# superlinear-ai/raglite

Measured on AMD Instinct MI355X. Metric: queries/sec, MaxSim 32x1M d=1024 exact top-100, higher is better.
Workload: dtype f32 in / f32 scores: candidate chunks found with the fp16 hi halves of corpus and queries (1 x v_mfma_f32_16x16x32_f16 per multiply, f32 accumulate, rigorous error bound), their scores by v_mfma_f32_16x16x4_f32 (exact f32 products); full-precision fallback: 3 x v_mfma_f32_16x16x32_f16 on hi+lo pairs

## Files before the change

include/raglite_hip.h:

```cpp
#ifndef RAGLITE_HIP_H
#define RAGLITE_HIP_H

#include <stddef.h>
#include <stdint.h>

#ifdef __cplusplus
extern "C" {
#endif

typedef enum {
    RL_OK = 0,
    RL_ERR_INVALID = -1,
    RL_ERR_HIP = -2,
    RL_ERR_UNSUPPORTED = -3,
    RL_ERR_NOMEM = -4
} rl_status;

typedef enum { RL_MEM_HOST = 0, RL_MEM_DEVICE = 1 } rl_mem;
typedef enum {
    RL_ARITH_AUTO = 0,
    RL_ARITH_FP32_EXACT = 1,
    RL_ARITH_F16_SPLIT = 2,
    RL_ARITH_F16_STORED = 3
} rl_arith;
// ... 36 lines not shown

#define RL_IMAGE_PRESPLIT 1u
#define RL_IMAGE_HI 2u
#define RL_IMAGE_HI_PLANE 4u
int rl_index_prepare(rl_index* index, uint32_t images, uint32_t* built, void* stream);

int rl_index_append(rl_index* index, const float* rows, int64_t n_new_rows, const int64_t* new_chunk_sizes,
                    int64_t n_new_chunks, int mem, void* stream);
int rl_index_delete_chunks(rl_index* index, const int64_t* chunk_ordinals, int64_t n, void* stream);
int rl_index_live(rl_index* index, int64_t* live_rows, int64_t* live_chunks, void* stream);
int rl_index_compact(rl_index* index, int64_t* out_remap, int64_t* new_n_rows, int64_t* new_n_chunks, void* stream);

int rl_index_set_arithmetic(rl_index* index, int mode);
int rl_index_arithmetic(rl_index* index, int* in_effect);

typedef enum {
    RL_OPT_HI_SEARCH = 1, RL_OPT_HI_MAXSIM = 2, RL_OPT_HI_PRODUCTS = 3, RL_OPT_PP_PASS = 4, RL_OPT_FUSED_TOPK = 5, RL_OPT_FUSED_HI = 6,
    RL_OPT_FUSED_PP = 7, RL_OPT_FUSED_TOPK_CAP = 8, RL_OPT_FUSED_TOPK_STRIDE = 9, RL_OPT_GEMM_PASS = 10, RL_OPT_QUERY_PAIRS = 11,
    RL_OPT_PLANES_GEMM = 12, RL_OPT_KEEP_IMAGE = 13, RL_OPT_KEEP_HI = 14, RL_OPT_IMAGE_HEADROOM_MB = 15, RL_OPT_ARITHMETIC = 16,
    RL_OPT_EXACT_KTH_THRESHOLD = 17, RL_OPT_FUSED_TWO_ROUNDS = 18, RL_OPT_KEEP_HI_PLANE = 19, RL_OPT_PAIRS_PACKED = 20,
    RL_OPT_F16_EXACT = 21, RL_OPT_LAZY_IMAGES = 22, RL_OPT_FUSED_PP_SAMPLE = 23,
    RL_OPT_LIST_SELECT = 24, RL_OPT_HI_FEW = 25, RL_OPT_TOPK_BLOCK = 26, RL_OPT_HI_PIVOT = 27, RL_OPT_COUNT_ = 28
} rl_option;
enum { RL_OPT_PP_SCHEDULE = 64 };
int rl_set_default_option(int key, int64_t value);
int rl_get_default_option(int key, int64_t* value);
int rl_index_set_option(rl_index* index, int key, int64_t value);
int rl_index_get_option(rl_index* index, int key, int64_t* value);

int rl_search_rows(rl_index* index, const float* queries, int32_t n_queries, int32_t k,
                   float* out_scores, int32_t* out_rows, int mem, void* stream);

int rl_rank_cut_begin(rl_index* index, const float* queries, int32_t n_queries, int mem, void* stream);
int rl_rank_cut_level(rl_index* index, int level, int64_t rank_limit, uint32_t* out_hist, int mem, void* stream);
int rl_rank_cut_level_done(rl_index* index, int level, const uint32_t* hist_sum, int mem, void* stream);
int rl_rank_cut_ties(rl_index* index, int64_t rank_limit, uint32_t* out_ties, int mem, void* stream);
int rl_rank_cut_finish(rl_index* index, int64_t rank_limit, const uint32_t* ties_before, const uint32_t* chunk_filter, int32_t k,
                       float* out_scores, int32_t* out_rows, int mem, void* stream);

int rl_search_chunks(rl_index* index, const float* queries, int32_t n_queries, int32_t num_hits,
                     int32_t k, float* out_scores, int32_t* out_chunks, int32_t* out_counts,
                     int mem, void* stream);

int rl_maxsim_topk(rl_index* index, const float* query_vecs, int32_t nq, int32_t k,
                   float* out_scores, int32_t* out_chunks, int mem, void* stream);
int rl_maxsim_scores(rl_index* index, const float* query_vecs, int32_t nq, float* out_scores,
                     int mem, void* stream);
// ... 106 lines not shown
```

raglite_amd/_abi.py:

```python

from __future__ import annotations

import ctypes as C
import functools
import os
from pathlib import Path

LIB_PATH = Path(os.environ.get("RAGLITE_HIP_LIB") or Path(__file__).resolve().parent / "_lib" / "libraglite_hip.so")

RL_OK, RL_ERR_INVALID, RL_ERR_HIP, RL_ERR_UNSUPPORTED, RL_ERR_NOMEM = 0, -1, -2, -3, -4
MEM_HOST, MEM_DEVICE = 0, 1
METRICS = {"cosine": 0, "dot": 1, "l2": 2}
SYNTH_KINDS = {"uniform": 0, "small_int": 1}
OPTIONS = {
    "hi_search": 1, "hi_maxsim": 2, "hi_products": 3, "pp_pass": 4, "fused_topk": 5, "fused_hi": 6, "fused_pp": 7, "fused_topk_cap": 8,
    "fused_topk_stride": 9, "gemm_pass": 10, "query_pairs": 11, "planes_gemm": 12, "keep_image": 13, "keep_hi": 14,
    "image_headroom_mb": 15, "arithmetic": 16, "exact_kth_threshold": 17, "fused_two_rounds": 18,
    "keep_hi_plane": 19, "pairs_packed": 20, "f16_exact": 21, "lazy_images": 22, "fused_pp_sample": 23, "list_select": 24, "hi_few": 25, "topk_block": 26, "hi_pivot": 27,
}
SCHEDULE_OPTIONS = {"pp_schedule": 64}


def option_key(name: str) -> int:
    return OPTIONS[name] if name in OPTIONS else SCHEDULE_OPTIONS[name]

c_void_p, c_int, c_i32, c_i64, c_u64, c_size_t = C.c_void_p, C.c_int, C.c_int32, C.c_int64, C.c_uint64, C.c_size_t
c_double, c_char_p = C.c_double, C.c_char_p

_SIGNATURES = {
    "rl_version": [],
    "rl_last_error": [],
    "rl_init": [c_int],
    "rl_device_count": [C.POINTER(c_int)],
    "rl_device_info": [c_int, c_char_p, c_int, C.POINTER(c_int), C.POINTER(c_i64)],
    "rl_dev_alloc": [C.POINTER(c_void_p), c_size_t],
    "rl_dev_free": [c_void_p],
    "rl_memcpy_h2d": [c_void_p, c_void_p, c_size_t, c_void_p],
    "rl_memcpy_d2h": [c_void_p, c_void_p, c_size_t, c_void_p],
    "rl_memcpy_d2d": [c_void_p, c_void_p, c_size_t, c_void_p],
    "rl_stream_sync": [c_void_p],
    "rl_synth_fill": [c_void_p, c_i64, c_i64, c_u64, c_int, c_void_p],
    "rl_pool_norm": [c_void_p, c_i64, c_i32, c_void_p, c_void_p, c_i64, c_i32, c_double, c_void_p, c_void_p,
                     c_int, c_void_p],
# ... 142 lines not shown
```

raglite_amd/csrc/api.hip:

```cpp
#include <cmath>
#include <cstdlib>
#include <cstring>
#include <limits>
#include <memory>
#include <mutex>
#include <utility>
#include <vector>

#include "common.h"

namespace rl {

static thread_local std::string g_last_error;
void set_error(const std::string& msg) { g_last_error = msg; }
int fail(int code, const std::string& msg) {
    g_last_error = msg;
    return code;
}

namespace {

hipStream_t as_stream(void* s) { return reinterpret_cast<hipStream_t>(s); }

struct BlockCache {
// ... 157 lines not shown
}
int sync_and_drain(hipStream_t s) {
    RL_HIP(hipStreamSynchronize(s));
    g_pinned.drain();
    return RL_OK;
}
int finish(int mem, hipStream_t s) {
    if (mem == RL_MEM_HOST) return sync_and_drain(s);
    return RL_OK;
}

int scan_mode(int metric) {
    switch (metric) {
        case RL_COSINE: return SCAN_COSINE;
        case RL_DOT: return SCAN_DOT;
        case RL_L2: return SCAN_L2;
        default: return -1;
    }
}

constexpr size_t SCORE_BATCH_BYTES = size_t(8) << 30;

struct Options {
    int64_t v[RL_OPT_PP_SCHEDULE + 1];
    Options() {
        for (auto& x : v) x = 0;
        v[RL_OPT_HI_SEARCH] = v[RL_OPT_HI_MAXSIM] = v[RL_OPT_HI_PRODUCTS] = v[RL_OPT_PP_PASS] = v[RL_OPT_FUSED_TOPK] = v[RL_OPT_FUSED_HI] = 1;
        v[RL_OPT_FUSED_PP] = v[RL_OPT_GEMM_PASS] = v[RL_OPT_QUERY_PAIRS] = v[RL_OPT_PLANES_GEMM] = v[RL_OPT_KEEP_IMAGE] = v[RL_OPT_KEEP_HI] = 1;
        v[RL_OPT_EXACT_KTH_THRESHOLD] = v[RL_OPT_FUSED_TWO_ROUNDS] = v[RL_OPT_KEEP_HI_PLANE] = v[RL_OPT_F16_EXACT] = v[RL_OPT_LAZY_IMAGES] = v[RL_OPT_FUSED_PP_SAMPLE] = v[RL_OPT_LIST_SELECT] = v[RL_OPT_HI_FEW] = 1;
        v[RL_OPT_TOPK_BLOCK] = v[RL_OPT_PAIRS_PACKED] = 2;
        v[RL_OPT_HI_PIVOT] = 1;
        v[RL_OPT_PP_SCHEDULE] = 1;
        v[RL_OPT_IMAGE_HEADROOM_MB] = -1;
        v[RL_OPT_ARITHMETIC] = RL_ARITH_AUTO;
    }
    bool on(int key) const { return v[key] != 0; }
};
std::mutex g_default_opts_mu;
Options g_default_opts;
bool option_key_ok(int key) { return (key >= 1 && key < RL_OPT_COUNT_) || key == RL_OPT_PP_SCHEDULE; }
bool option_value_ok(int key, int64_t value) {
    switch (key) {
        case RL_OPT_HI_SEARCH: case RL_OPT_HI_MAXSIM: case RL_OPT_PP_PASS: case RL_OPT_FUSED_TOPK: case RL_OPT_FUSED_HI: case RL_OPT_FUSED_PP:
        case RL_OPT_GEMM_PASS: case RL_OPT_QUERY_PAIRS: case RL_OPT_PLANES_GEMM: case RL_OPT_KEEP_IMAGE: case RL_OPT_KEEP_HI:
        case RL_OPT_EXACT_KTH_THRESHOLD: case RL_OPT_FUSED_TWO_ROUNDS: case RL_OPT_KEEP_HI_PLANE: case RL_OPT_F16_EXACT: case RL_OPT_LAZY_IMAGES: case RL_OPT_FUSED_PP_SAMPLE: case RL_OPT_LIST_SELECT: case RL_OPT_HI_FEW: case RL_OPT_HI_PIVOT:
        case RL_OPT_PP_SCHEDULE:
            return value == 0 || value == 1;
        case RL_OPT_TOPK_BLOCK: case RL_OPT_PAIRS_PACKED: return value >= 0 && value <= 2;
        case RL_OPT_HI_PRODUCTS: return value == 1 || value == 2;
        case RL_OPT_FUSED_TOPK_CAP: return value >= 0 && value <= MERGE_CAP;
        case RL_OPT_FUSED_TOPK_STRIDE: return value == 0 || (value >= 2 && value <= (int64_t(1) << 20));
        case RL_OPT_IMAGE_HEADROOM_MB: return value >= -1 && value <= (int64_t(1) << 30);
        case RL_OPT_ARITHMETIC: return value == RL_ARITH_AUTO || value == RL_ARITH_FP32_EXACT;
        default: return false;
    }
}

struct Image {
    Pool buf;
    float scale = 0.f;
    int64_t rows = 0;
    void drop() {
        buf.release();
        scale = 0.f;
        rows = 0;
    }
    bool covers(float at, int64_t n_rows) const { return scale > 0.f && scale == at && rows == n_rows && n_rows > 0; }
};
struct NormStats {
    float max_row_norm = 0.f, max_lo_norm = 0.f, max_lo_ratio = 0.f;
// ... 1740 lines not shown
    hb.m = hb.es + (size_t)n * hb.cap;
    hb.es_top = hb.m + n;
    hb.bmax = reinterpret_cast<uint64_t*>((reinterpret_cast<uintptr_t>(hb.es_top + (size_t)n * k) + 7) & ~uintptr_t(7));
}
size_t hi_batch_words(int32_t n, int32_t k) {
    return (size_t)n * k * 3 + (size_t)n * 3 + 16 + (size_t)n * 2048 * 2 + 2 + 2 * pivot_scratch_words(std::min<int32_t>(n, 2));
}
int hi_batch_approx(rl_index* idx, const float* d_q, int32_t nq, int32_t n_queries, int32_t n_gemm, int32_t k, float* sc, int64_t ld, HiBatch& hb,
                    hipStream_t s, bool flag_zeroed = false) {
    hb.one_product = idx->opt.v[RL_OPT_HI_PRODUCTS] == 1;
    hb.exact_kth = idx->opt.on(RL_OPT_EXACT_KTH_THRESHOLD);
    RL_TRY(idx->hibuf.reserve(hi_batch_words(n_gemm, k) * 4));
    hi_batch_layout(idx, n_gemm, k, hb);
    const int32_t cap = hb.cap;
    hb.m_abs = idx->norm_stats.max_lo_norm + sum_eps(idx->dim) * idx->norm_stats.max_row_norm;
    hb.q_unscale = reinterpret_cast<const float*>(idx->qplanes.as<char>() + (size_t)n_queries * idx->dim * 128);
    hb.qsum = hb.q_unscale + 2 * (size_t)n_queries;
    if (!flag_zeroed) RL_HIP(hipMemsetAsync(hb.flag, 0, 16 * sizeof(uint32_t), s));
    (void)cap;
    const bool pp = hb.one_product && idx->dim >= 256 && idx->opt.on(RL_OPT_PP_PASS);
    if (pp)
        RL_TRY(launch_maxsim_pp(approx_image(idx), idx->n_rows, idx->dim, idx->qplanes.p, n_queries, 0, n_gemm, nq, idx->row_to_chunk,
                                idx->offsets, idx->ends.as<uint32_t>(), sc, ld, idx->n_cu, s, approx_scale(idx), nullptr,
                                (int)idx->opt.v[RL_OPT_PP_SCHEDULE]));
    for (int32_t b = 0; !pp && b < n_gemm; b += GEMM_PASS_QUERIES) {
        const int32_t n_q = std::min<int32_t>(GEMM_PASS_QUERIES, n_gemm - b);
        RL_TRY(launch_maxsim_gemm(approx_image(idx), idx->n_rows, idx->dim, idx->qplanes.p, n_queries, b, n_q, nq, idx->row_to_chunk,
                                  idx->offsets, idx->ends.as<uint32_t>(), sc + (int64_t)b * ld, ld, idx->n_cu, s, approx_scale(idx), true,
                                  nullptr, hb.one_product));
    }
    RL_TRY(mask_chunk_scores(idx, sc, n_gemm, ld, hb.filter, s));
    int st_pv = RL_ERR_UNSUPPORTED;
    if (n_gemm < 16 && idx->n_chunks > (int64_t)262144 && idx->opt.on(RL_OPT_HI_PIVOT))
        st_pv = launch_topk_pivot(sc, n_gemm, idx->n_chunks, ld, k, idx->ws, hb.ts, hb.ti, s);
    if (st_pv != RL_OK && st_pv != RL_ERR_UNSUPPORTED) return st_pv;
    if (st_pv == RL_ERR_UNSUPPORTED) RL_TRY(launch_topk(sc, n_gemm, idx->n_chunks, ld, k, idx->ws, hb.ts, hb.ti, s));
    return RL_OK;
}
int hi_batch_fallback(rl_index* idx, const float* d_q, int32_t nq, int32_t n_queries, int32_t n_gemm, int32_t k, float* sc, int64_t ld,
                      const HiBatch& hb, float* d_s, int32_t* d_c, hipStream_t s, bool rows_only = false);
int hi_batch_rescore(rl_index* idx, const float* d_q, int32_t nq, int32_t n_queries, int32_t n_gemm, int32_t k, float* sc, int64_t ld,
                     const HiBatch& hb, float* d_s, int32_t* d_c, hipStream_t s, bool rows_only = false) {
    const size_t q_elems = (size_t)nq * idx->dim;
    const float* rows = idx->E16 ? reinterpret_cast<const float*>(idx->E16) : idx->E;
    const bool rows16 = idx->E16 != nullptr;
    idx->filt = {RL_FILTER_MAXSIM_BATCH, n_gemm, hb.cap, hb.cnt, hb.flag};
    const int packed = (int)idx->opt.v[RL_OPT_PAIRS_PACKED];
// ... 321 lines not shown
    hipStream_t s = as_stream(stream);
    std::lock_guard<std::mutex> lock(idx->mu);
    RL_TRY(use_scratch(idx, s));
    if (idx->has_empty_chunk || idx->n_chunks == 0)
        return fail(RL_ERR_UNSUPPORTED, "rl_maxsim_approx_scores: the approximate pass needs an index without empty chunks");
    RL_TRY(demand_images(idx, approx_image_bit(idx), s));
    if (!approx_image_valid(idx) || nq > 32 || (kernel == 0 && idx->dim < 256))
        return fail(RL_ERR_UNSUPPORTED, "rl_maxsim_approx_scores: this index keeps no HI image (or nq > 32 / dim < 256)");
    DevBuf t_q, t_o, t_b;
    const float* d_q; float* d_o; float* d_b = nullptr;
    const size_t q_elems = (size_t)nq * idx->dim;
    const int64_t ld = idx->n_chunks;
    RL_TRY(stage_in(query_vecs, (size_t)n_queries * q_elems, mem, s, t_q, &d_q));
    RL_TRY(stage_out_begin(out_scores, (size_t)n_queries * ld, mem, t_o, &d_o));
    if (out_bound) RL_TRY(stage_out_begin(out_bound, (size_t)n_queries, mem, t_b, &d_b));
    RL_TRY(idx->qplanes.reserve(query_planes_bytes(idx->dim, n_queries)));
    RL_TRY(launch_query_planes(d_q, idx->dim, nq, (int64_t)q_elems, n_queries, idx->qplanes.p, s));
    const int32_t per = kernel == 0 ? n_queries : GEMM_PASS_QUERIES;
    for (int32_t b = 0; b < n_queries; b += per) {
        const int32_t n_q = std::min<int32_t>(per, n_queries - b);
        if (kernel == 0)
            RL_TRY(launch_maxsim_pp(approx_image(idx), idx->n_rows, idx->dim, idx->qplanes.p, n_queries, b, n_q, nq, idx->row_to_chunk, idx->offsets,
                                    idx->ends.as<uint32_t>(), d_o + (int64_t)b * ld, ld, idx->n_cu, s, approx_scale(idx), nullptr,
                                    (int)idx->opt.v[RL_OPT_PP_SCHEDULE]));
        else
            RL_TRY(launch_maxsim_gemm(approx_image(idx), idx->n_rows, idx->dim, idx->qplanes.p, n_queries, b, n_q, nq, idx->row_to_chunk, idx->offsets,
                                      idx->ends.as<uint32_t>(), d_o + (int64_t)b * ld, ld, idx->n_cu, s, approx_scale(idx), true, nullptr, true));
    }
    if (d_b) {
        const float m_abs = idx->norm_stats.max_lo_norm + sum_eps(idx->dim) * idx->norm_stats.max_row_norm;
        const float* q_unscale = reinterpret_cast<const float*>(idx->qplanes.as<char>() + (size_t)n_queries * idx->dim * 128);
        RL_TRY(idx->hibuf.reserve((size_t)n_queries * 4 * sizeof(float) + 64));
        float* top = idx->hibuf.as<float>();
        float* thr = top + n_queries;
        uint32_t* cnt = reinterpret_cast<uint32_t*>(thr + n_queries);
        uint32_t* flag = cnt + n_queries;
        RL_HIP(hipMemsetAsync(top, 0, (size_t)n_queries * sizeof(float), s));
        RL_HIP(hipMemsetAsync(flag, 0, 16 * sizeof(uint32_t), s));
        RL_TRY(launch_maxsim_threshold(top, n_queries, 1, d_q, nq, idx->dim, (int64_t)q_elems, 1.0f, m_abs, thr, cnt, flag, s, q_unscale,
                                       idx->norm_stats.max_row_norm + idx->norm_stats.max_lo_norm));
        RL_TRY(launch_scale_f32(thr, d_b, -0.5f, n_queries, s));
        idx->filt = {};
    }
    RL_TRY(stage_out_end(out_scores, (size_t)n_queries * ld, mem, s, t_o));
    if (out_bound) RL_TRY(stage_out_end(out_bound, (size_t)n_queries, mem, s, t_b));
    return finish(mem, s);
}
// ... 182 lines not shown
    int st = RL_OK;
    if (kind == 2) {
        st = pairs_prepare(idx, q_dev, nq / 2, (int64_t)(nq / 2) * idx->dim, 2, s);
        if (st != RL_OK) { (void)hipEventDestroy(e0); (void)hipEventDestroy(e1); return st == RL_ERR_UNSUPPORTED ? fail(st, "rl_time_kernel: the pair kernel does not apply to this index / shape") : st; }
    }
    if (kind == 3 || kind == 5 || kind == 6) {
        st = gemm_prepare(idx, q_dev, nq / GEMM_PASS_QUERIES, (int64_t)(nq / GEMM_PASS_QUERIES) * idx->dim, GEMM_PASS_QUERIES, s, true);
        if (st == RL_OK && !image_valid(idx)) st = RL_ERR_UNSUPPORTED;
        if (st != RL_OK) { (void)hipEventDestroy(e0); (void)hipEventDestroy(e1); return st == RL_ERR_UNSUPPORTED ? fail(st, "rl_time_kernel: the eight-query kernel does not apply to this index / shape") : st; }
    }
    if (kind == 7) {
        st = pp_vec >= 1 && pp_vec * pp_n == nq ? gemm_prepare(idx, q_dev, pp_vec, (int64_t)pp_vec * idx->dim, pp_n, s) : RL_ERR_UNSUPPORTED;
        if (st == RL_OK && !(approx_image_valid(idx) && idx->dim >= 256)) st = RL_ERR_UNSUPPORTED;
        if (st != RL_OK) { (void)hipEventDestroy(e0); (void)hipEventDestroy(e1); return st == RL_ERR_UNSUPPORTED ? fail(st, "rl_time_kernel: the sixteen-query kernel does not apply to this index / shape") : st; }
    }
    if (kind == 4 || kind == 10) {
        st = demand_images(idx, IMG_HI_PLANE, s);
        if (st != RL_OK) { (void)hipEventDestroy(e0); (void)hipEventDestroy(e1); return st; }
    }
    RL_HIP(hipEventRecord(e0, s));
    for (int i = 0; i < iters && st == RL_OK; ++i) {
        if (kind == 7) st = launch_maxsim_pp(approx_image(idx), idx->n_rows, idx->dim, idx->qplanes.p, pp_n, 0, pp_n,
                                             pp_vec, idx->row_to_chunk, idx->offsets, idx->ends.as<uint32_t>(), idx->scores.as<float>(), ldc,
                                             idx->n_cu, s, approx_scale(idx), nullptr, (int)idx->opt.v[RL_OPT_PP_SCHEDULE]);
        else if (kind == 3) st = gemm_pass(idx, nq / GEMM_PASS_QUERIES, GEMM_PASS_QUERIES, 0, GEMM_PASS_QUERIES, idx->scores.as<float>(), ldc, s);
        else if (kind == 8) {
            const auto& r = idx->replay;
            if (hipMemsetAsync(r.cnt, 0, (size_t)r.B * sizeof(uint32_t), s) != hipSuccess) st = RL_ERR_HIP;
            else if (r.pp && r.round1_tiles > 0) {
                CandArgs ca1 = r.ca;
                ca1.tau = r.thr1;
                st = launch_pp_rows_pass(idx->hi_image.buf.p, idx->n_rows, idx->dim, r.B, r.qs, idx->norm, r.mode, &ca1, idx->pp_work.p, r.log_cap, idx->n_cu, s,
                                         idx->split_scale, 0, r.round1_tiles, false, r.row_test);
                if (st == RL_OK)
                    st = launch_pp_rows_pass(idx->hi_image.buf.p, idx->n_rows, idx->dim, r.B, r.qs, idx->norm, r.mode, &r.ca, idx->pp_work.p, r.log_cap, idx->n_cu, s,
                                             idx->split_scale, r.round1_tiles, -1, true, r.row_test);
            }
            else if (r.pp) st = launch_pp_rows_pass(idx->hi_image.buf.p, idx->n_rows, idx->dim, r.B, r.qs, idx->norm, r.mode, &r.ca, idx->pp_work.p, r.log_cap,
                                                    idx->n_cu, s, idx->split_scale, 0, -1, false, r.row_test);
            else st = launch_score_planes_pass(idx->hi_image.buf.p, idx->n_rows, idx->dim, r.B, r.qs, nullptr, 0, idx->norm, idx->sumsq, r.mode, 1, nullptr, &r.ca,
                                               idx->n_cu, s, idx->split_scale, true, true);
        }
        else if (kind == 0) st = maxsim_scores_device(idx, q_dev, nq, idx->scores.as<float>(), s);
        else if (kind == 9) st = launch_mfma_f16_rate(idx->scores.as<float>(), idx->n_cu, MFMA_RATE_ITERS, s, nullptr);
        else if (kind == 2) st = pairs_pass(idx, nq / 2, 2, 0, idx->scores.as<float>(), ldc, s);
        else if (kind == 5 || kind == 6) {
            st = hi_image_valid(idx) ? launch_maxsim_gemm(idx->hi_image.buf.p, idx->n_rows, idx->dim, idx->qplanes.p, GEMM_PASS_QUERIES, 0,
// ... 418 lines not shown
```

raglite_amd/csrc/common.h:

```cpp
#pragma once
#include <hip/hip_runtime.h>
#include <stdint.h>

#include <algorithm>
#include <cstdlib>
#include <string>

#include "raglite_hip.h"

namespace rl {

void set_error(const std::string& msg);
int fail(int code, const std::string& msg);

#define RL_HIP(expr)                                                                         \
    do {                                                                                     \
        hipError_t _e = (expr);                                                              \
        if (_e != hipSuccess)                                                                \
            return ::rl::fail(_e == hipErrorOutOfMemory ? RL_ERR_NOMEM : RL_ERR_HIP,         \
                              std::string(#expr) + ": " + hipGetErrorString(_e));            \
    } while (0)

#define RL_TRY(expr)              \
    do {                          \
// ... 298 lines not shown
                               int64_t out_stride, int n_cu, hipStream_t s, float split_scale, const uint32_t* run_if = nullptr);
size_t query_split_bytes(int32_t dim, int32_t n_queries);
int launch_query_split(const float* Q, int32_t dim, int32_t nq, int64_t q_stride, int32_t n_queries, void* buf, bool f16_corpus,
                       hipStream_t s);
int launch_maxsim_stream2(const void* D, bool f16, int64_t n_rows, int32_t dim, const void* split_buf, int32_t n_queries,
                          int32_t first, int32_t nq, const int32_t* row_to_chunk, const int64_t* chunk_offsets, int64_t n_chunks,
                          float* out, int64_t out_stride, int n_cu, hipStream_t s, float split_scale);
size_t planes_bytes(int64_t rows, int32_t dim, bool half = false);
int launch_presplit_rows(const float* E, int64_t first_row, int64_t n_rows, int32_t dim, float scale, void* planes, hipStream_t s);
int launch_preformat_rows16(const uint16_t* E, int64_t first_row, int64_t n_rows, int32_t dim, void* planes, hipStream_t s);
int launch_presplit_hi_rows(const float* E, int64_t first_row, int64_t n_rows, int32_t dim, float scale, void* planes, hipStream_t s);
size_t chunk_ends_words(int64_t rows);
int launch_chunk_ends(const int32_t* row_to_chunk, int64_t n_rows, uint32_t* ends, hipStream_t s);
size_t query_planes_bytes(int32_t dim, int32_t n_queries);
int launch_query_planes(const float* Q, int32_t dim, int32_t nq, int64_t q_stride, int32_t n_queries, void* buf, hipStream_t s,
                        uint32_t* zero_words = nullptr, int n_zero = 0);
int launch_maxsim_gemm(const void* planes, int64_t n_rows, int32_t dim, const void* qbuf, int32_t n_queries, int32_t first,
                       int32_t n_q, int32_t nq, const int32_t* row_to_chunk, const int64_t* chunk_offsets, const uint32_t* ends_bits,
                       float* out, int64_t out_stride, int n_cu, hipStream_t s, float split_scale, bool half = false,
                       const uint32_t* run_if = nullptr, bool hi_only = false, bool all_passes = false);
constexpr int32_t PP_PASS_QUERIES = 16;
int launch_maxsim_pp(const void* image, int64_t n_rows, int32_t dim, const void* qbuf, int32_t n_queries, int32_t first, int32_t n_q,
                     int32_t nq, const int32_t* row_to_chunk, const int64_t* chunk_offsets, const uint32_t* ends_bits, float* out,
                     int64_t out_stride, int n_cu, hipStream_t s, float split_scale, const uint32_t* run_if, int schedule);
constexpr int32_t MFMA_RATE_ITERS = 1000;
int launch_mfma_f16_rate(float* out, int n_cu, int32_t iters, hipStream_t s, double* flops);
size_t score_planes_scratch_floats(int32_t nb, int32_t dim);
int launch_score_planes(const void* planes, int64_t n_rows, int32_t dim, const float* Q, int32_t nb, float* scores, int64_t ld,
                        const float* row_norm, const float* row_sumsq, float* scratch, int mode, int n_cu, hipStream_t s, float split_scale,
                        bool half = false);
struct CandArgs { const float* tau; int32_t tau_stride; float* scores; int32_t* ids; uint32_t* cnt; uint32_t* overflow; int32_t cap; };
int launch_score_planes_queries(const float* Q, int32_t nb, int32_t dim, float* scratch, int mode, hipStream_t s, uint32_t* zero_word = nullptr);
size_t pp_rows_scratch_bytes(int64_t n_rows, int32_t nb, int n_cu, int32_t expected_per_query, int32_t* log_cap_out);
int launch_pp_rows_pass(const void* image, int64_t n_rows, int32_t dim, int32_t nb, float* scratch, const float* row_norm, int mode,
                        const CandArgs* cand, void* work, int32_t log_cap, int n_cu, hipStream_t s, float split_scale, int64_t tile_begin = 0,
                        int64_t tile_count = -1, bool norms_ready = false,
                        bool row_norm_test = false);
int launch_pp_rows_sample(const void* image, int64_t n_rows, int32_t dim, int32_t nb, float* scratch, const float* row_norm, int mode, float* S,
                          int64_t ld_s, int32_t stride, int n_cu, hipStream_t s, float split_scale);
int launch_raise_threshold(float* thr, const float* kth, int32_t nq, int32_t k, const float* window, hipStream_t s);
int launch_score_planes_pass(const void* planes, int64_t n_rows, int32_t dim, int32_t nb, float* scratch, float* scores, int64_t ld,
                             const float* row_norm, const float* row_sumsq, int mode, int32_t tile_stride, const uint32_t* run_if,
                             const CandArgs* cand, int n_cu, hipStream_t s, float split_scale, bool half = false, bool hi_only = false);
int launch_row_range(const float* E, int64_t n_rows, int32_t dim, uint32_t* range, hipStream_t s);
int launch_score_gemm(const float* E, int64_t n_rows, int32_t dim, const float* Q, int32_t nb, float* scores,
                      int64_t ld, const float* row_norm, const float* row_sumsq, float* q_sumsq_scratch, int mode,
                      int n_cu, hipStream_t s, float split_scale = 0.f);
// ... 24 lines not shown
```

raglite_amd/csrc/maxsim_pp.hip:

```cpp
#include <cstdio>
#include <cstdlib>
#include <utility>

#include "common.h"
#include "pp_schedule.h"

namespace rl {

typedef float f32x4 __attribute__((ext_vector_type(4)));
typedef _Float16 h16x8 __attribute__((ext_vector_type(8)));

namespace {
constexpr int PP_RT = 128;
constexpr int PP_NBLK = PP_RT / 16;
constexpr int PP_QPP = 16;
constexpr int PP_DC = 8;
constexpr int PP_LC = 6;
constexpr int PP_CSLOT = PP_NBLK * 1024;
constexpr int PP_STAGE = 1536;
constexpr int PP_LDS = PP_DC * PP_CSLOT + 16 * PP_STAGE * 4;

__device__ __forceinline__ int64_t pp_uniform_i64(int64_t v) {
    const uint32_t lo = __builtin_amdgcn_readfirstlane((uint32_t)(uint64_t)v);
    const uint32_t hi = __builtin_amdgcn_readfirstlane((uint32_t)((uint64_t)v >> 32));
    return (int64_t)(((uint64_t)hi << 32) | lo);
}

template <bool NT>
__device__ __forceinline__ void pp_dma(uint32_t lds, const char* src, uint32_t lane16) {
    const uint32_t l = __builtin_amdgcn_readfirstlane(lds);
    const char* const p = reinterpret_cast<const char*>(pp_uniform_i64(reinterpret_cast<int64_t>(src)));
    if constexpr (NT)
        asm volatile("s_mov_b32 m0, %0\n\ts_nop 0\n\tglobal_load_lds_dwordx4 %1, %2 nt" ::"s"(l), "v"(lane16), "s"(p) : "memory", "m0");
    else
        asm volatile("s_mov_b32 m0, %0\n\ts_nop 0\n\tglobal_load_lds_dwordx4 %1, %2" ::"s"(l), "v"(lane16), "s"(p) : "memory", "m0");
}

template <int OFF>
__device__ __forceinline__ void pp_read(f32x4& dst, uint32_t addr) {
    asm volatile("ds_read_b128 %0, %1 offset:%2" : "=v"(dst) : "v"(addr), "n"(OFF) : "memory");
}
__device__ __forceinline__ void pp_pin(f32x4& a, f32x4& b, f32x4& c, f32x4& d) { asm volatile("" : "+v"(a), "+v"(b), "+v"(c), "+v"(d)); }
typedef float f32x16s __attribute__((ext_vector_type(16)));
__device__ __forceinline__ f32x16s pp_sload16(const float* p) {
    f32x16s v;
    const float* const u = reinterpret_cast<const float*>(pp_uniform_i64(reinterpret_cast<int64_t>(p)));
    asm volatile("s_load_dwordx16 %0, %1, 0x0\n\ts_waitcnt lgkmcnt(0)" : "=s"(v) : "s"(u) : "memory");
    return v;
}
__device__ __forceinline__ h16x8 pp_h(const f32x4& v) {
    h16x8 r;
    __builtin_memcpy(&r, &v, 16);
    return r;
}
}

struct PpRows {
    const float* tau;
    const float* q_unscale;
    const float* q_sumsq;
    const float* row_norm;
    const float* blk_minmax;
    int32_t B, QT, metric;
    float* cand_scores; int32_t* cand_ids; uint32_t* cand_cnt; uint32_t* overflow; int32_t cap;
    uint2* log; int32_t log_cap;
    int32_t tile_begin, tile_count;
    float* S; int64_t ld_s; int32_t stride;
};

template <int DBG, int MODE, bool ROWNORM>
__global__ __launch_bounds__(512, 2) void maxsim_pp_kernel(const char* __restrict__ planes, int64_t n_rows, int32_t nslab,
                                                           const char* __restrict__ qfrag, const float* __restrict__ qmeta, int32_t n_q,
                                                           const int32_t* __restrict__ row_to_chunk, const int64_t* __restrict__ chunk_offsets,
                                                           const uint32_t* __restrict__ ends_bits, float* __restrict__ out, int64_t out_stride,
                                                           float inv_e_scale, const uint32_t* __restrict__ run_if, PpRows rs) {
    constexpr bool ROWS = MODE == 2, SCORES = MODE == 1, GROUPS = ROWS || SCORES;
    __shared__ __attribute__((aligned(16))) char smem[PP_LDS];
    if (run_if && __builtin_amdgcn_readfirstlane((int)*run_if) == 0) return;
    const int lane = threadIdx.x & 63;
    const int wv = wave_id();
    int64_t G = gridDim.x, b = blockIdx.x;
    int qt = (int)blockIdx.y;
    if constexpr (!GROUPS) {
        const PpSlot m = pp_schedule((int32_t)blockIdx.x, (int32_t)blockIdx.y, (int32_t)gridDim.x, (int32_t)gridDim.y, (n_q + PP_QPP - 1) / PP_QPP);
        G = m.ranges;
        b = m.range;
        qt = m.pass;
    }
    auto boundary = [&](int64_t t) -> int64_t {
        if (t <= 0) return 0;
        if (t >= n_rows) return n_rows;
        const int32_t c = row_to_chunk[t];
        const int64_t c0 = chunk_offsets[c], c1 = chunk_offsets[c + 1];
        return c0 == t ? t : c1;
    };
    int32_t r_lo = 0, r_hi = 0, nt_rows = 0;
    if constexpr (!GROUPS) {
        r_lo = (int32_t)pp_uniform_i64(boundary((n_rows * b) / G));
        r_hi = (int32_t)pp_uniform_i64((b + 1 == G) ? n_rows : boundary((n_rows * (b + 1)) / G));
        if (r_hi <= r_lo) return;
    } else {
        const int64_t Tr = rs.tile_count;
        const int64_t t0 = (Tr * b) / G, t1 = (Tr * (b + 1)) / G;
        nt_rows = (int32_t)(t1 - t0);
        if (nt_rows <= 0) return;
        r_lo = (int32_t)((rs.tile_begin + t0) * PP_RT);
        r_hi = (int32_t)n_rows;
    }
    const int32_t org = r_lo & ~15;
    const int nt = GROUPS ? nt_rows : (r_hi - org + PP_RT - 1) / PP_RT;
// ... 10 lines not shown
    const int32_t last_blk = (int32_t)((n_rows + 15) >> 4) - 1;
    const uint32_t lds_base = (uint32_t)reinterpret_cast<uintptr_t>((__attribute__((address_space(3))) char*)smem);
    const uint32_t lane16 = 16u * lane;

    const bool has0 = q_base + 2 * wv < n_q, has1 = q_base + 2 * wv + 1 < n_q;
    int ql0 = PP_QPP * qt + 2 * wv, ql1 = PP_QPP * qt + 2 * wv + 1;
    ql0 = ql0 < n_q ? ql0 : n_q - 1;
    ql1 = ql1 < n_q ? ql1 : n_q - 1;
    const char* const qp0 = qfrag + pp_uniform_i64((int64_t)ql0 * nslab * 4096);
    const char* const qp1 = qfrag + pp_uniform_i64((int64_t)ql1 * nslab * 4096);
    int qr_s = 0;
    auto issue_qregs = [&](f32x4 (&qn)[4]) __attribute__((always_inline)) {
        if constexpr (!(DBG & 32)) {
            const char* const a0 = reinterpret_cast<const char*>(pp_uniform_i64(reinterpret_cast<int64_t>(qp0 + (int64_t)qr_s * 4096)));
            const char* const a1 = reinterpret_cast<const char*>(pp_uniform_i64(reinterpret_cast<int64_t>(qp1 + (int64_t)qr_s * 4096)));
            asm volatile("global_load_dwordx4 %0, %2, %3\n\tglobal_load_dwordx4 %1, %2, %3 offset:2048"
                         : "=&v"(qn[0]), "=&v"(qn[1]) : "v"(lane16), "s"(a0) : "memory");
            asm volatile("global_load_dwordx4 %0, %2, %3\n\tglobal_load_dwordx4 %1, %2, %3 offset:2048"
                         : "=&v"(qn[2]), "=&v"(qn[3]) : "v"(lane16), "s"(a1) : "memory");
            if (++qr_s == nslab) qr_s = 0;
        }
    };
    int fc_s = 0, fc_r = 0, fc_slot = 0;
    const int32_t blk_org = (org >> 4) + wv;
    const int64_t slab_bytes = (int64_t)nslab * 1024;
    auto issue_c = [&]() __attribute__((always_inline)) {
        if constexpr (!(DBG & 16)) {
            const int t = fc_r < nt ? fc_r : nt - 1;
            int32_t blk = SCORES ? tile_blk(t) + wv : blk_org + t * PP_NBLK;
            blk = blk < last_blk ? blk : last_blk;
            const char* src = planes + pp_uniform_i64((int64_t)blk * slab_bytes + (int64_t)fc_s * 1024);
            pp_dma<GROUPS>(lds_base + (uint32_t)(fc_slot * PP_CSLOT + wv * 1024), src, lane16);
        }
        if (++fc_s == nslab) { fc_s = 0; ++fc_r; }
        fc_slot = fc_slot + 1 == PP_DC ? 0 : fc_slot + 1;
    };

    f32x4 acc[2][2][PP_NBLK];
#pragma unroll
    for (int q = 0; q < 2; ++q)
#pragma unroll
        for (int qb = 0; qb < 2; ++qb)
#pragma unroll
            for (int a = 0; a < PP_NBLK; ++a) acc[q][qb][a] = (f32x4){0.f, 0.f, 0.f, 0.f};

    f32x4 ef[PP_NBLK];
    f32x4 qA[4], qB[4];
    int c_slot = 0;
    const uint32_t rd_c = lds_base + lane16;
    auto read_slab = [&](auto A_) __attribute__((always_inline)) {
        constexpr int a = decltype(A_)::value;
        if constexpr (!(DBG & 8)) pp_read<a * 1024>(ef[a], rd_c + (uint32_t)(c_slot * PP_CSLOT));
    };
    auto mfma_group = [&](f32x4 (&q)[4], auto A_) __attribute__((always_inline)) {
        constexpr int A = decltype(A_)::value;
// ... 428 lines not shown
#undef PP_I
    if (wv < 4) main_loop(std::false_type{});
    else main_loop(std::true_type{});
    asm volatile("s_waitcnt vmcnt(0)" ::: "memory");
    dump_log();
    flush_rows();
    flush_out();
    if constexpr (DBG & 128) {
        if (n_q > 1000000) {
            f32x4 t = (f32x4){0.f, 0.f, 0.f, 0.f};
#pragma unroll
            for (int q = 0; q < 2; ++q)
#pragma unroll
                for (int qb = 0; qb < 2; ++qb)
#pragma unroll
                    for (int a = 0; a < PP_NBLK; ++a) t += acc[q][qb][a];
            out[lane] = (t[0] + t[1]) + (t[2] + t[3]);
        }
    }
}

int launch_maxsim_pp(const void* image, int64_t n_rows, int32_t dim, const void* qbuf, int32_t n_queries, int32_t first, int32_t n_q,
                     int32_t nq, const int32_t* row_to_chunk, const int64_t* chunk_offsets, const uint32_t* ends_bits, float* out,
                     int64_t out_stride, int n_cu, hipStream_t s, float split_scale, const uint32_t* run_if, int schedule) {
    if (nq < 1 || nq > 32 || n_q < 1 || n_q > PP_QPP * 4096 || n_rows < 1 || first < 0 || first + n_q > n_queries) return RL_ERR_UNSUPPORTED;
    if (dim % 32 || dim < 256 || !(split_scale > 0.f) || !image || !ends_bits) return RL_ERR_UNSUPPORTED;
    const int32_t nslab = dim / 32;
    const char* qfrag = static_cast<const char*>(qbuf) + (size_t)first * nslab * 4096;
    const float* qmeta = reinterpret_cast<const float*>(static_cast<const char*>(qbuf) + (size_t)n_queries * dim * 128) + 2 * (size_t)first;
    const int64_t tiles = (n_rows + PP_RT - 1) / PP_RT;
    const int64_t gx = std::max<int64_t>(1, std::min<int64_t>(n_cu > 0 ? n_cu : 256, tiles)), passes = (n_q + PP_QPP - 1) / PP_QPP;
    const dim3 grid = schedule == 1 ? dim3((unsigned)(gx * passes)) : dim3((unsigned)gx, (unsigned)passes), blk(512);
#define RL_PP_LAUNCH(DBG_)                                                                                                                 \
    hipLaunchKernelGGL((maxsim_pp_kernel<DBG_, 0, false>), grid, blk, 0, s, static_cast<const char*>(image), n_rows, nslab, qfrag, qmeta, n_q, row_to_chunk, \
                       chunk_offsets, ends_bits, out, out_stride, 1.0f / split_scale, run_if, PpRows{})
#ifdef RAGLITE_EXPERIMENTS
    static const int dbg = std::getenv("RAGLITE_PP_DBG") ? std::atoi(std::getenv("RAGLITE_PP_DBG")) : 0;
    if (dbg == 2) RL_PP_LAUNCH(2);
    else if (dbg == 128) RL_PP_LAUNCH(128);
    else if (dbg == 136) RL_PP_LAUNCH(136);
    else if (dbg == 144) RL_PP_LAUNCH(144);
    else if (dbg == 160) RL_PP_LAUNCH(160);
    else if (dbg == 184) RL_PP_LAUNCH(184);
    else RL_PP_LAUNCH(0);
#else
    RL_PP_LAUNCH(0);
#endif
#undef RL_PP_LAUNCH
    RL_HIP(hipGetLastError());
    return RL_OK;
}

__global__ __launch_bounds__(256) void block_norm_minmax_kernel(const float* __restrict__ row_norm, int64_t n_rows, int64_t n_blocks,
                                                                 float* __restrict__ out) {
    const int64_t blk = (int64_t)blockIdx.x * 256 + threadIdx.x;
    if (blk >= n_blocks) return;
    float mn = INFINITY, mx = 0.f;
    for (int i = 0; i < 16; ++i) {
        const int64_t r = blk * 16 + i;
// ... 142 lines not shown
```

raglite_amd/csrc/pp_schedule.h:

```cpp
#pragma once
#include <stdint.h>

#if defined(__HIPCC__) || defined(__CUDACC__)
#define RL_PP_HD __host__ __device__
#else
#define RL_PP_HD
#endif

namespace rl {

struct PpSlot {
    int32_t ranges;
    int32_t range;
    int32_t pass;
};

RL_PP_HD inline PpSlot pp_schedule(int32_t x, int32_t y, int32_t gx, int32_t gy, int32_t passes) {
    if (gy > 1 || passes <= 1) return PpSlot{gx, x, y};
    const int32_t ranges = gx / passes;
    const int32_t whole = ranges & ~7, head = whole * passes;
    if (x < head) return PpSlot{ranges, 8 * (x / (8 * passes)) + x % 8, (x / 8) % passes};
    const int32_t t = x - head, rest = ranges - whole;
    return PpSlot{ranges, whole + t % rest, t / rest};
}

}
```

Before: 17650.

## Add XCD-affine block-to-(range,pass) schedule for the MaxSim PP kernel

```diff
diff --git a/include/raglite_hip.h b/include/raglite_hip.h
--- a/include/raglite_hip.h
+++ b/include/raglite_hip.h
@@ -82,7 +82,7 @@
     RL_OPT_F16_EXACT = 21, RL_OPT_LAZY_IMAGES = 22, RL_OPT_FUSED_PP_SAMPLE = 23,
     RL_OPT_LIST_SELECT = 24, RL_OPT_HI_FEW = 25, RL_OPT_TOPK_BLOCK = 26, RL_OPT_HI_PIVOT = 27, RL_OPT_COUNT_ = 28
 } rl_option;
-enum { RL_OPT_PP_SCHEDULE = 64 };
+enum { RL_OPT_PP_SCHEDULE = 64, RL_OPT_PP_XCD_PASSES = 65 };
 int rl_set_default_option(int key, int64_t value);
 int rl_get_default_option(int key, int64_t* value);
 int rl_index_set_option(rl_index* index, int key, int64_t value);
diff --git a/raglite_amd/_abi.py b/raglite_amd/_abi.py
--- a/raglite_amd/_abi.py
+++ b/raglite_amd/_abi.py
@@ -18,7 +18,7 @@
     "image_headroom_mb": 15, "arithmetic": 16, "exact_kth_threshold": 17, "fused_two_rounds": 18,
     "keep_hi_plane": 19, "pairs_packed": 20, "f16_exact": 21, "lazy_images": 22, "fused_pp_sample": 23, "list_select": 24, "hi_few": 25, "topk_block": 26, "hi_pivot": 27,
 }
-SCHEDULE_OPTIONS = {"pp_schedule": 64}
+SCHEDULE_OPTIONS = {"pp_schedule": 64, "pp_xcd_passes": 65}
 
 
 def option_key(name: str) -> int:
diff --git a/raglite_amd/csrc/api.hip b/raglite_amd/csrc/api.hip
--- a/raglite_amd/csrc/api.hip
+++ b/raglite_amd/csrc/api.hip
@@ -203,7 +203,7 @@
 constexpr size_t SCORE_BATCH_BYTES = size_t(8) << 30;
 
 struct Options {
-    int64_t v[RL_OPT_PP_SCHEDULE + 1];
+    int64_t v[RL_OPT_PP_XCD_PASSES + 1];
     Options() {
         for (auto& x : v) x = 0;
         v[RL_OPT_HI_SEARCH] = v[RL_OPT_HI_MAXSIM] = v[RL_OPT_HI_PRODUCTS] = v[RL_OPT_PP_PASS] = v[RL_OPT_FUSED_TOPK] = v[RL_OPT_FUSED_HI] = 1;
@@ -212,6 +212,7 @@
         v[RL_OPT_TOPK_BLOCK] = v[RL_OPT_PAIRS_PACKED] = 2;
         v[RL_OPT_HI_PIVOT] = 1;
         v[RL_OPT_PP_SCHEDULE] = 1;
+        v[RL_OPT_PP_XCD_PASSES] = 2;
         v[RL_OPT_IMAGE_HEADROOM_MB] = -1;
         v[RL_OPT_ARITHMETIC] = RL_ARITH_AUTO;
     }
@@ -219,7 +220,7 @@
 };
 std::mutex g_default_opts_mu;
 Options g_default_opts;
-bool option_key_ok(int key) { return (key >= 1 && key < RL_OPT_COUNT_) || key == RL_OPT_PP_SCHEDULE; }
+bool option_key_ok(int key) { return (key >= 1 && key < RL_OPT_COUNT_) || key == RL_OPT_PP_SCHEDULE || key == RL_OPT_PP_XCD_PASSES; }
 bool option_value_ok(int key, int64_t value) {
     switch (key) {
         case RL_OPT_HI_SEARCH: case RL_OPT_HI_MAXSIM: case RL_OPT_PP_PASS: case RL_OPT_FUSED_TOPK: case RL_OPT_FUSED_HI: case RL_OPT_FUSED_PP:
@@ -227,6 +228,7 @@
         case RL_OPT_EXACT_KTH_THRESHOLD: case RL_OPT_FUSED_TWO_ROUNDS: case RL_OPT_KEEP_HI_PLANE: case RL_OPT_F16_EXACT: case RL_OPT_LAZY_IMAGES: case RL_OPT_FUSED_PP_SAMPLE: case RL_OPT_LIST_SELECT: case RL_OPT_HI_FEW: case RL_OPT_HI_PIVOT:
         case RL_OPT_PP_SCHEDULE:
             return value == 0 || value == 1;
+        case RL_OPT_PP_XCD_PASSES: return value == 8 || value == 4 || value == 2 || value == 1;
         case RL_OPT_TOPK_BLOCK: case RL_OPT_PAIRS_PACKED: return value >= 0 && value <= 2;
         case RL_OPT_HI_PRODUCTS: return value == 1 || value == 2;
         case RL_OPT_FUSED_TOPK_CAP: return value >= 0 && value <= MERGE_CAP;
@@ -2013,7 +2015,7 @@
     if (pp)
         RL_TRY(launch_maxsim_pp(approx_image(idx), idx->n_rows, idx->dim, idx->qplanes.p, n_queries, 0, n_gemm, nq, idx->row_to_chunk,
                                 idx->offsets, idx->ends.as<uint32_t>(), sc, ld, idx->n_cu, s, approx_scale(idx), nullptr,
-                                (int)idx->opt.v[RL_OPT_PP_SCHEDULE]));
+                                (int)idx->opt.v[RL_OPT_PP_SCHEDULE], (int)idx->opt.v[RL_OPT_PP_XCD_PASSES]));
     for (int32_t b = 0; !pp && b < n_gemm; b += GEMM_PASS_QUERIES) {
         const int32_t n_q = std::min<int32_t>(GEMM_PASS_QUERIES, n_gemm - b);
         RL_TRY(launch_maxsim_gemm(approx_image(idx), idx->n_rows, idx->dim, idx->qplanes.p, n_queries, b, n_q, nq, idx->row_to_chunk,
@@ -2381,7 +2383,7 @@
         if (kernel == 0)
             RL_TRY(launch_maxsim_pp(approx_image(idx), idx->n_rows, idx->dim, idx->qplanes.p, n_queries, b, n_q, nq, idx->row_to_chunk, idx->offsets,
                                     idx->ends.as<uint32_t>(), d_o + (int64_t)b * ld, ld, idx->n_cu, s, approx_scale(idx), nullptr,
-                                    (int)idx->opt.v[RL_OPT_PP_SCHEDULE]));
+                                    (int)idx->opt.v[RL_OPT_PP_SCHEDULE], (int)idx->opt.v[RL_OPT_PP_XCD_PASSES]));
         else
             RL_TRY(launch_maxsim_gemm(approx_image(idx), idx->n_rows, idx->dim, idx->qplanes.p, n_queries, b, n_q, nq, idx->row_to_chunk, idx->offsets,
                                       idx->ends.as<uint32_t>(), d_o + (int64_t)b * ld, ld, idx->n_cu, s, approx_scale(idx), true, nullptr, true));
@@ -2610,7 +2612,7 @@
     for (int i = 0; i < iters && st == RL_OK; ++i) {
         if (kind == 7) st = launch_maxsim_pp(approx_image(idx), idx->n_rows, idx->dim, idx->qplanes.p, pp_n, 0, pp_n,
                                              pp_vec, idx->row_to_chunk, idx->offsets, idx->ends.as<uint32_t>(), idx->scores.as<float>(), ldc,
-                                             idx->n_cu, s, approx_scale(idx), nullptr, (int)idx->opt.v[RL_OPT_PP_SCHEDULE]);
+                                             idx->n_cu, s, approx_scale(idx), nullptr, (int)idx->opt.v[RL_OPT_PP_SCHEDULE], (int)idx->opt.v[RL_OPT_PP_XCD_PASSES]);
         else if (kind == 3) st = gemm_pass(idx, nq / GEMM_PASS_QUERIES, GEMM_PASS_QUERIES, 0, GEMM_PASS_QUERIES, idx->scores.as<float>(), ldc, s);
         else if (kind == 8) {
             const auto& r = idx->replay;
diff --git a/raglite_amd/csrc/common.h b/raglite_amd/csrc/common.h
--- a/raglite_amd/csrc/common.h
+++ b/raglite_amd/csrc/common.h
@@ -344,7 +344,7 @@
 constexpr int32_t PP_PASS_QUERIES = 16;
 int launch_maxsim_pp(const void* image, int64_t n_rows, int32_t dim, const void* qbuf, int32_t n_queries, int32_t first, int32_t n_q,
                      int32_t nq, const int32_t* row_to_chunk, const int64_t* chunk_offsets, const uint32_t* ends_bits, float* out,
-                     int64_t out_stride, int n_cu, hipStream_t s, float split_scale, const uint32_t* run_if, int schedule);
+                     int64_t out_stride, int n_cu, hipStream_t s, float split_scale, const uint32_t* run_if, int schedule, int xcd_passes);
 constexpr int32_t MFMA_RATE_ITERS = 1000;
 int launch_mfma_f16_rate(float* out, int n_cu, int32_t iters, hipStream_t s, double* flops);
 size_t score_planes_scratch_floats(int32_t nb, int32_t dim);
diff --git a/raglite_amd/csrc/maxsim_pp.hip b/raglite_amd/csrc/maxsim_pp.hip
--- a/raglite_amd/csrc/maxsim_pp.hip
+++ b/raglite_amd/csrc/maxsim_pp.hip
@@ -26,11 +26,20 @@
     return (int64_t)(((uint64_t)hi << 32) | lo);
 }
 
+enum { PP_HINT_NONE = 0, PP_HINT_NT = 1, PP_HINT_SC1 = 2 };
 template <bool NT>
-__device__ __forceinline__ void pp_dma(uint32_t lds, const char* src, uint32_t lane16) {
+__device__ __forceinline__ void pp_dma(uint32_t lds, const char* src, uint32_t lane16, int hint) {
     const uint32_t l = __builtin_amdgcn_readfirstlane(lds);
     const char* const p = reinterpret_cast<const char*>(pp_uniform_i64(reinterpret_cast<int64_t>(src)));
+#ifdef RAGLITE_EXPERIMENTS
+    if (!NT && hint == PP_HINT_SC1) {
+        asm volatile("s_mov_b32 m0, %0\n\ts_nop 0\n\tglobal_load_lds_dwordx4 %1, %2 sc1" ::"s"(l), "v"(lane16), "s"(p) : "memory", "m0");
+        return;
+    }
+    if (NT || hint == PP_HINT_NT)
+#else
     if constexpr (NT)
+#endif
         asm volatile("s_mov_b32 m0, %0\n\ts_nop 0\n\tglobal_load_lds_dwordx4 %1, %2 nt" ::"s"(l), "v"(lane16), "s"(p) : "memory", "m0");
     else
         asm volatile("s_mov_b32 m0, %0\n\ts_nop 0\n\tglobal_load_lds_dwordx4 %1, %2" ::"s"(l), "v"(lane16), "s"(p) : "memory", "m0");
@@ -66,6 +75,7 @@
     uint2* log; int32_t log_cap;
     int32_t tile_begin, tile_count;
     float* S; int64_t ld_s; int32_t stride;
+    int32_t xcd_passes, dma_hint;
 };
 
 template <int DBG, int MODE, bool ROWNORM>
@@ -82,10 +92,12 @@
     int64_t G = gridDim.x, b = blockIdx.x;
     int qt = (int)blockIdx.y;
     if constexpr (!GROUPS) {
-        const PpSlot m = pp_schedule((int32_t)blockIdx.x, (int32_t)blockIdx.y, (int32_t)gridDim.x, (int32_t)gridDim.y, (n_q + PP_QPP - 1) / PP_QPP);
-        G = m.ranges;
-        b = m.range;
-        qt = m.pass;
+        const int32_t passes = (n_q + PP_QPP - 1) / PP_QPP;
+        const PpSlot m = gridDim.y > 1 ? pp_schedule((int32_t)blockIdx.x, (int32_t)blockIdx.y, (int32_t)gridDim.x, (int32_t)gridDim.y, passes)
+                                       : pp_schedule_affine((int32_t)blockIdx.x, (int32_t)gridDim.x, passes, rs.xcd_passes);
+        G = __builtin_amdgcn_readfirstlane(m.ranges);
+        b = __builtin_amdgcn_readfirstlane(m.range);
+        qt = __builtin_amdgcn_readfirstlane(m.pass);
     }
     auto boundary = [&](int64_t t) -> int64_t {
         if (t <= 0) return 0;
@@ -142,6 +154,7 @@
         }
     };
     int fc_s = 0, fc_r = 0, fc_slot = 0;
+    const int dma_hint = GROUPS ? 0 : rs.dma_hint;
     const int32_t blk_org = (org >> 4) + wv;
     const int64_t slab_bytes = (int64_t)nslab * 1024;
     auto issue_c = [&]() __attribute__((always_inline)) {
@@ -150,7 +163,7 @@
             int32_t blk = SCORES ? tile_blk(t) + wv : blk_org + t * PP_NBLK;
             blk = blk < last_blk ? blk : last_blk;
             const char* src = planes + pp_uniform_i64((int64_t)blk * slab_bytes + (int64_t)fc_s * 1024);
-            pp_dma<GROUPS>(lds_base + (uint32_t)(fc_slot * PP_CSLOT + wv * 1024), src, lane16);
+            pp_dma<GROUPS>(lds_base + (uint32_t)(fc_slot * PP_CSLOT + wv * 1024), src, lane16, dma_hint);
         }
         if (++fc_s == nslab) { fc_s = 0; ++fc_r; }
         fc_slot = fc_slot + 1 == PP_DC ? 0 : fc_slot + 1;
@@ -625,7 +638,7 @@
 
 int launch_maxsim_pp(const void* image, int64_t n_rows, int32_t dim, const void* qbuf, int32_t n_queries, int32_t first, int32_t n_q,
                      int32_t nq, const int32_t* row_to_chunk, const int64_t* chunk_offsets, const uint32_t* ends_bits, float* out,
-                     int64_t out_stride, int n_cu, hipStream_t s, float split_scale, const uint32_t* run_if, int schedule) {
+                     int64_t out_stride, int n_cu, hipStream_t s, float split_scale, const uint32_t* run_if, int schedule, int xcd_passes) {
     if (nq < 1 || nq > 32 || n_q < 1 || n_q > PP_QPP * 4096 || n_rows < 1 || first < 0 || first + n_q > n_queries) return RL_ERR_UNSUPPORTED;
     if (dim % 32 || dim < 256 || !(split_scale > 0.f) || !image || !ends_bits) return RL_ERR_UNSUPPORTED;
     const int32_t nslab = dim / 32;
@@ -634,10 +647,14 @@
     const int64_t tiles = (n_rows + PP_RT - 1) / PP_RT;
     const int64_t gx = std::max<int64_t>(1, std::min<int64_t>(n_cu > 0 ? n_cu : 256, tiles)), passes = (n_q + PP_QPP - 1) / PP_QPP;
     const dim3 grid = schedule == 1 ? dim3((unsigned)(gx * passes)) : dim3((unsigned)gx, (unsigned)passes), blk(512);
+    PpRows rs{};
+    rs.xcd_passes = schedule == 1 ? xcd_passes : 8;
 #define RL_PP_LAUNCH(DBG_)                                                                                                                 \
     hipLaunchKernelGGL((maxsim_pp_kernel<DBG_, 0, false>), grid, blk, 0, s, static_cast<const char*>(image), n_rows, nslab, qfrag, qmeta, n_q, row_to_chunk, \
-                       chunk_offsets, ends_bits, out, out_stride, 1.0f / split_scale, run_if, PpRows{})
+                       chunk_offsets, ends_bits, out, out_stride, 1.0f / split_scale, run_if, rs)
 #ifdef RAGLITE_EXPERIMENTS
+    const int force_hint = std::getenv("RAGLITE_PP_HINT") ? std::atoi(std::getenv("RAGLITE_PP_HINT")) : -1;
+    if (force_hint >= PP_HINT_NONE && force_hint <= PP_HINT_SC1) rs.dma_hint = force_hint;
     static const int dbg = std::getenv("RAGLITE_PP_DBG") ? std::atoi(std::getenv("RAGLITE_PP_DBG")) : 0;
     if (dbg == 2) RL_PP_LAUNCH(2);
     else if (dbg == 128) RL_PP_LAUNCH(128);
diff --git a/raglite_amd/csrc/pp_schedule.h b/raglite_amd/csrc/pp_schedule.h
--- a/raglite_amd/csrc/pp_schedule.h
+++ b/raglite_amd/csrc/pp_schedule.h
@@ -24,4 +24,20 @@
     return PpSlot{ranges, whole + t % rest, t / rest};
 }
 
+RL_PP_HD inline int32_t pp_affine_blocks(int32_t ranges, int32_t passes, int32_t w) {
+    return ((w == 1 || w == 2 || w == 4) && ranges > 0 && ranges % w == 0) ? passes / 8 : 0;
 }
+RL_PP_HD inline PpSlot pp_schedule_affine(int32_t x, int32_t gx, int32_t passes, int32_t w) {
+    const int32_t ranges = passes > 0 ? gx / passes : gx;
+    const int32_t blocks = pp_affine_blocks(ranges, passes, w), head = 8 * ranges * blocks;
+    if (blocks == 0) return pp_schedule(x, 0, gx, 1, passes);
+    if (x >= head) {
+        const int32_t rest = passes - 8 * blocks;
+        const PpSlot m = pp_schedule(x - head, 0, ranges * rest, 1, rest);
+        return PpSlot{ranges, m.range, 8 * blocks + m.pass};
+    }
+    const int32_t S = 8 / w, blk = x / (8 * ranges), l = x % (8 * ranges), slot = l % 8, n = l / 8, s = slot % S, j = slot / S;
+    return PpSlot{ranges, w * (n / w) + j, 8 * blk + w * s + n % w};
+}
+
+}
```

Result: faster. 18020 (median of 6 runs) (+2.1%).
